# vocdoni/zk-franchise-proof-circuit

Measured on AMD Instinct MI355X. Metric: zkCensus proofs/sec (nLevels=160), higher is better.
Workload: dtype u256 (8 x u32 Montgomery, BN254 Fr/Fq)

## Files before the change

### include/zkcensus.h

```cpp
#ifndef ZKCENSUS_H
#define ZKCENSUS_H
#include <stddef.h>
#include <stdint.h>
#ifdef __cplusplus
extern "C" {
#endif

typedef struct zkc_ctx zkc_ctx;
typedef struct zkc_zkey zkc_zkey;

enum {
    ZKC_OK = 0,
    ZKC_ERR_GENERIC = 1,
    ZKC_ERR_SHORT_BUFFER = 2,
    ZKC_ERR_INVALID_WITNESS_LENGTH = 3,
    ZKC_ERR_BAD_ARG = 4,
    ZKC_ERR_FORMAT = 5,
    ZKC_ERR_HIP = 6,
    ZKC_ERR_WITNESS = 7
};
enum {
    ZKC_W_OK = 0, ZKC_W_ERR_WEIGHT = 1 , ZKC_W_ERR_SIK_ROOT = 2 ,
    ZKC_W_ERR_CENSUS_ROOT = 3 , ZKC_W_ERR_NULLIFIER = 4 , ZKC_W_ERR_LAST_SIBLING = 5 ,
    ZKC_W_ERR_INPUT_RANGE = 6 ,
// ... 5 lines not shown
void zkc_ctx_destroy(zkc_ctx* ctx);
const char* zkc_last_error(const zkc_ctx* ctx);
void* zkc_ctx_stream(zkc_ctx* ctx);

int zkc_circuit_n_inputs(int nLevels);
int zkc_circuit_n_wires(int nLevels);
int zkc_circuit_nlevels_from_wasm(const void* wasm, size_t len, char sha256_hex[65]);
void zkc_sha256(const void* data, size_t len, uint8_t out[32]);

int zkc_witness(zkc_ctx* ctx, int nLevels, const void* inputs, int B, void* wtns, int32_t* status);
int zkc_inputs_from_json(const char* json, size_t len, int nLevels, void* out, char* err, size_t errlen);
int zkc_witness_dev(zkc_ctx* ctx, int nLevels, const void* d_inputs, int B, void* d_wtns, int32_t* d_status );

int  zkc_zkey_load(zkc_ctx* ctx, const void* zkey_bytes, size_t len, zkc_zkey** out);
void zkc_zkey_free(zkc_zkey* zk);
int  zkc_zkey_info(const zkc_zkey* zk, uint32_t* nVars, uint32_t* nPublic, uint32_t* domainSize);
int  zkc_zkey_pass_info(const zkc_zkey* zk, int* pass_size, int* lanes);
int  zkc_zkey_header_info(const void* zkey_bytes, size_t len, uint32_t* nVars, uint32_t* nPublic, uint32_t* domainSize);
int  zkc_zkey_sha256(const zkc_zkey* zk, uint8_t out[32]);
int  zkc_zkey_fingerprint(const void* zkey_bytes, size_t len, uint8_t out[32]);

void zkc_random_scalars(uint8_t* out, size_t n);
int zkc_prove(zkc_zkey* zk, const void* wtns, uint32_t nWitness, const uint8_t r[32], const uint8_t s[32],
              uint8_t proof[256], uint8_t* public_out);
int zkc_prove_dev(zkc_zkey* zk, const void* d_wtns, uint32_t nWitness, const uint8_t r[32], const uint8_t s[32],
                  uint8_t proof[256], uint8_t* public_out);

int zkc_prove_batch_dev(zkc_zkey* zk, const void* d_wtns, uint32_t nWitness, int B, const uint8_t* rs, uint8_t* proofs, uint8_t* publics);

int zkc_fullprove_batch_dev(zkc_zkey* zk, const void* d_inputs, int B, void* d_wtns, int32_t* d_status, const uint8_t* rs, uint8_t* proofs, uint8_t* publics);
// ... 130 lines not shown
```

### zk-franchise-proof-circuit_amd/__init__.py

```python
import ctypes
from . import _native
from ._native import ZkcError
from .inputs import INPUT_KEYS, flatten_inputs, R_MOD

__all__ = ['Context', 'ProvingKey', 'DevicePool', 'ProvingService', 'groth16', 'ZkcError', 'INPUT_KEYS', 'flatten_inputs', 'R_MOD']


class Context:

    def __init__(self, device=0):
        self._lib = _native.load()
        h = ctypes.c_void_p()
        rc = self._lib.zkc_ctx_create(int(device), ctypes.byref(h))
        if rc != 0:
            raise ZkcError(rc, (self._lib.zkc_last_error(None) or b'').decode())
        self._h = h
        self.device = device
        self._keys = []

    def close(self):
        if getattr(self, '_h', None):
            for k in list(self._keys):
                k.close()
            self._lib.zkc_ctx_destroy(self._h)
# ... 37 lines not shown
class ProvingKey:

    def __init__(self, ctx, zkey_bytes):
        self.ctx = ctx
        self._lib = ctx._lib
        h = ctypes.c_void_p()
        ctx._check(self._lib.zkc_zkey_load(ctx._h, zkey_bytes, len(zkey_bytes), ctypes.byref(h)))
        self._h = h
        ctx._keys.append(self)
        a, b, c = ctypes.c_uint32(), ctypes.c_uint32(), ctypes.c_uint32()
        self._lib.zkc_zkey_info(h, ctypes.byref(a), ctypes.byref(b), ctypes.byref(c))
        self.n_vars, self.n_public, self.domain_size = a.value, b.value, c.value
        ps, ln = ctypes.c_int(), ctypes.c_int()
        self._lib.zkc_zkey_pass_info(h, ctypes.byref(ps), ctypes.byref(ln))
        self.pass_size, self.lanes = ps.value, ln.value

    def close(self):
        if getattr(self, '_h', None):
            if getattr(self.ctx, '_h', None):
                self._lib.zkc_zkey_free(self._h)
            self._h = None
            if self in self.ctx._keys:
                self.ctx._keys.remove(self)

    def __del__(self):
        try:
            self.close()
        except Exception:
            pass

# ... 152 lines not shown
```

### zk-franchise-proof-circuit_amd/_native.py

```python
import ctypes
import os

_HERE = os.path.dirname(os.path.abspath(__file__))
LIB_PATH = os.environ.get('ZKCENSUS_LIB') or os.path.join(_HERE, 'libzkcensus.so')
_lib = None


class ZkcError(RuntimeError):
    def __init__(self, code, msg):
        super().__init__('libzkcensus error %d: %s' % (code, msg))
        self.code = code


def load():
    global _lib
    if _lib is not None:
        return _lib
    if not os.path.exists(LIB_PATH):
        raise ImportError('libzkcensus.so is not built (run `python -c "import __graft_entry__ as g; g.build()"`); '
                          'there is no CPU fallback for the product path')
    try:
        import torch
    except ImportError:
        pass
    L = ctypes.CDLL(LIB_PATH)
    vp, i32p = ctypes.c_void_p, ctypes.POINTER(ctypes.c_int32)
    L.zkc_ctx_create.argtypes = [ctypes.c_int, ctypes.POINTER(vp)]
    L.zkc_ctx_destroy.argtypes = [vp]
    L.zkc_last_error.argtypes = [vp]; L.zkc_last_error.restype = ctypes.c_char_p
    L.zkc_ctx_stream.argtypes = [vp]; L.zkc_ctx_stream.restype = vp
    L.zkc_witness.argtypes = [vp, ctypes.c_int, vp, ctypes.c_int, vp, i32p]
    L.zkc_witness_dev.argtypes = [vp, ctypes.c_int, vp, ctypes.c_int, vp, vp]
    u8p, u32p = ctypes.c_char_p, ctypes.POINTER(ctypes.c_uint32)
    L.zkc_zkey_load.argtypes = [vp, ctypes.c_char_p, ctypes.c_size_t, ctypes.POINTER(vp)]
    L.zkc_zkey_free.argtypes = [vp]; L.zkc_zkey_free.restype = None
    L.zkc_zkey_info.argtypes = [vp, u32p, u32p, u32p]
    L.zkc_zkey_pass_info.argtypes = [vp, ctypes.POINTER(ctypes.c_int), ctypes.POINTER(ctypes.c_int)]
    L.zkc_witness_status_text.argtypes = [ctypes.c_int, ctypes.c_int32]; L.zkc_witness_status_text.restype = ctypes.c_char_p
    L.zkc_prove.argtypes = [vp, ctypes.c_char_p, ctypes.c_uint32, u8p, u8p, ctypes.c_char_p, ctypes.c_char_p]
    L.zkc_prove_dev.argtypes = [vp, vp, ctypes.c_uint32, u8p, u8p, ctypes.c_char_p, ctypes.c_char_p]
    L.zkc_prove_batch_dev.argtypes = [vp, vp, ctypes.c_uint32, ctypes.c_int, ctypes.c_char_p, ctypes.c_char_p, ctypes.c_char_p]
    L.zkc_fullprove_batch_dev.argtypes = [vp, vp, ctypes.c_int, vp, vp, ctypes.c_char_p, ctypes.c_char_p, ctypes.c_char_p]
    L.zkc_debug_stage.argtypes = [vp, vp, ctypes.c_int, ctypes.c_char_p]
    L.zkc_debug_early_retries.argtypes = []; L.zkc_debug_early_retries.restype = ctypes.c_ulonglong
    L.zkc_msm_debug.argtypes = [vp, ctypes.c_int, vp, ctypes.c_uint32, ctypes.c_char_p]
    L.zkc_debug_pairing_dev.argtypes = [vp, ctypes.c_char_p, ctypes.c_char_p, ctypes.c_char_p, ctypes.c_int, ctypes.c_char_p, ctypes.c_char_p, i32p, ctypes.POINTER(ctypes.c_int),
                                        ctypes.POINTER(ctypes.c_uint32), ctypes.c_size_t, ctypes.c_char_p]
    ulp = ctypes.POINTER(ctypes.c_ulong)
    L.groth16_prover.argtypes = [ctypes.c_char_p, ctypes.c_ulong, ctypes.c_char_p, ctypes.c_ulong, ctypes.c_char_p, ulp, ctypes.c_char_p, ulp, ctypes.c_char_p, ctypes.c_ulong]
    L.zkc_verify.argtypes = [ctypes.c_char_p, ctypes.c_char_p, ctypes.c_char_p]
    L.zkc_verify_bin.argtypes = [ctypes.c_char_p, ctypes.c_int, ctypes.c_char_p, ctypes.c_char_p]
    L.zkc_verify_batch.argtypes = [vp, ctypes.c_char_p, ctypes.c_int, ctypes.c_char_p, ctypes.c_char_p, ctypes.c_int, ctypes.c_char_p]
# ... 114 lines not shown
```

### zk-franchise-proof-circuit_amd/csrc/zkc_pass_plan.h

```cpp
#pragma once
#include "zkc_top_fold.h"
#include <cstddef>
#include <cstdint>
#include <vector>

namespace zkc {
constexpr int MSM_C_G2_LONE = 8;
constexpr int msm_nw(int c) { return (254 + c) / c; }
constexpr int msm_half(int c) { return 1 << (c - 1); }

namespace plan {

struct CallSplit { int npasses, per_pass; };
inline CallSplit call_split(int B, int max_inflight) {
    const int npasses = (B + max_inflight - 1) / max_inflight;
    return {npasses, (B + npasses - 1) / npasses};
}

constexpr int FOREIGN = -1;
inline int row_depth(const uint32_t* f, int n) {
    if (f[n - 1]) return FOREIGN;
    int D = 0; for (int g = 0; g < n - 1; g++) if (f[g]) D = g + 1;
    return D;
}
// ... 20 lines not shown
        if (!listed) seeds.push_back({q, t, slot});
    }
}

struct KeyShape {
    int c_sec, c_h, c_deep;
    uint32_t nv, np, n;
    uint32_t offA, offB1, offC, offA_deep, offB1_deep, offC_deep;
    bool lone_table, fb4;
};
struct LaneCaps { size_t w1_entries, w1_buckets; int w1_jobs; size_t w2_entries; };
struct Switches {
    uint32_t vw_big = 0, vw_small = 0, vw_g2 = 0; size_t deep_wires = 16000;
    bool matvec_inline = false, g2_acc_hold = false, g2_acc_early = false, reduce_stream = false;
    bool serial_streams = false;
};
struct PassShape {
    uint32_t vws, vwb, vw_g2;
    bool deep; int cw;
    uint32_t oA, oB1, oC;
    int c2;
    bool tree; int per;
};
template <class Lists> inline PassShape pass_shape(const KeyShape& k, int nb, const Lists* lists, const LaneCaps& cap, const Switches& s) {
    const uint32_t nv = k.nv, nc = nv - k.np - 1;
    PassShape p;
    p.vws = nb <= 4 ? 64u : s.vw_small ? s.vw_small : nb < 32 ? 256u : 2048u; p.vwb = nb <= 4 ? 256u : s.vw_big ? s.vw_big : nb < 32 ? 1024u : 4096u;
    size_t lone_entries = 0; for (int q = 0; q < nb; q++) lone_entries += (size_t)msm_nw(MSM_C_G2_LONE) * (lists ? lists[q].nB : nv);
    size_t live_wires = 0; for (int q = 0; q < nb; q++) live_wires += lists ? (size_t)lists[q].nA + lists[q].nB + lists[q].nC : 2 * (size_t)nv + nc;
    p.deep = k.c_deep != 0 && nb > 2 && live_wires >= 3 * s.deep_wires * (size_t)nb;
// ... 20 lines not shown
    bool mv_done;
    bool g2_acc_with_sort;
    bool red_split;
    bool blind_on_st;
};
inline StreamOrder stream_order(int nb, bool one_lane, int pass, int npasses, int lane0, bool tree, const Switches& s) {
    StreamOrder o;
    o.mv_prefetch = !s.matvec_inline && one_lane;
    o.mv_done = o.mv_prefetch && pass > 0;
    o.g2_acc_with_sort = s.g2_acc_hold || ((nb < 32 || !one_lane) && !s.g2_acc_early);
    o.red_split = s.reduce_stream && !s.serial_streams && nb >= 32;
    o.blind_on_st = (tree || lane0 >= 0) && npasses == 1;
    return o;
}

}}
```

### zk-franchise-proof-circuit_amd/csrc/zkc_prove.hip

```cpp
#include "zkc_prover.h"
#include "zkc_fixedbase.h"
#include "zkc_hostparse.h"
#include "zkc_host_util.h"
#include "zkc_kernels.h"
#include "zkc_f29_g2.h"
#include <cstring>
#include <ctime>
#include <cstdio>
#include <algorithm>
#include <atomic>

using namespace zkc;

void zkc::matvec_launch(zkc_zkey* zk, Fr* d_abc, Fr* d_wm, const uint32_t* d_wtns0, int nb, hipStream_t mv, const zkc_zkey::Fold::AbcRows* al) {
    const uint32_t n = zk->n, nv = zk->nVars;
    const bool units = zk->n_unit_coeffs > 0 && nv <= 3 * (size_t)n && sw::on<sw::ZKC_MATVEC_UNITS>();
    const Fr* wm = units ? (const Fr*)d_wm : (const Fr*)nullptr;
    if (al) {
        const uint32_t per = 6 * n;
        hipLaunchKernelGGL(zkc_abc_fill, dim3((per + 1023) / 1024, nb), dim3(256), 0, mv, (const uint4*)zk->fold.d_abc_tmpl, (uint4*)d_abc, per);
        if (units && al->nW) hipLaunchKernelGGL(zkc_wtns_mont_list, dim3((al->nW + 255) / 256, nb), dim3(256), 0, mv, (const Fr*)d_wtns0, (size_t)nv, d_wm, 3 * (size_t)n, al->d + al->offW, al->nW);
        if (al->nrows) hipLaunchKernelGGL(zkc_matvec_jds, dim3((al->nrows + 63 * al->nlong + 255) / 256, nb), dim3(256), 0, mv, zk->d_perm, zk->d_rowlen, zk->d_jdptr, zk->d_col, zk->d_val,
                                          (const Fr*)d_wtns0, (size_t)nv, d_abc, (int)n, al->nlong, wm, 3 * (size_t)n, (const uint32_t*)al->d, al->nrows);
        if (al->nC) hipLaunchKernelGGL(zkc_pointwise_mul, dim3((al->nC + 255) / 256, nb), dim3(256), 0, mv, d_abc, (int)n, (const uint32_t*)(al->d + al->offC), al->nC);
// ... 57 lines not shown
        lane_release(L);
        for (hipEvent_t e : {L.ev_msm, L.ev_msm2, L.ev_sorted, L.ev_ntt, L.ev_mv, L.ev_acc, L.ev_fin[0], L.ev_fin[1], L.ev_red}) if (e) (void)hipEventDestroy(e);
    }
    delete[] ctx->lanes; ctx->lanes = nullptr;
}
static int lane_init(zkc_ctx* ctx, int l) {
    zkc_lane& L = ctx_lanes(ctx)[l];
    if (L.made) return ZKC_OK;
    zkc_ctx::LaneStreams ls; int rc = zkc_lane_streams(ctx, l, sw::on<sw::ZKC_REDUCE_STREAM>(), &ls); if (rc) return rc;
    L.st = ls.st; L.st2 = ls.st2; L.fin = ls.fin; L.red = ls.red;
    for (hipEvent_t* e : {&L.ev_msm, &L.ev_msm2, &L.ev_sorted, &L.ev_ntt, &L.ev_mv, &L.ev_acc, &L.ev_fin[0], &L.ev_fin[1], &L.ev_red}) if (!*e) ZKC_HIP_CHECK(ctx, hipEventCreateWithFlags(e, hipEventDisableTiming));
    L.made = true; return ZKC_OK;
}
struct LaneSt { hipStream_t st, st2, fin, red; };
static LaneSt lane_st(const zkc_zkey* zk, const zkc_lane& L) { hipStream_t c = zk->ctx->stream; return zk->serial_streams ? LaneSt{c, c, c, c} : LaneSt{L.st, L.st2, L.fin, L.red}; }
static int lane_ensure(zkc_zkey* zk, int l, int inflight) {
    zkc_ctx* ctx = zk->ctx; int rc;
    if ((rc = lane_init(ctx, l))) return rc;
    zkc_lane& L = ctx->lanes[l];
    inflight = std::max(1, std::min(inflight, zk->max_inflight));
    if (lane_holds(L, lane_need(zk, inflight))) return ZKC_OK;
    inflight = std::min(inflight <= 4 ? 4 : zk->max_inflight, zk->max_inflight);
    LaneNeed nd = lane_need(zk, inflight);
    nd.abc = std::max(nd.abc, L.cap_abc); nd.p = std::max(nd.p, L.cap_p); nd.fin = std::max(nd.fin, L.cap_fin); nd.bs = std::max(nd.bs, L.cap_bs);
    nd.e1 = std::max(nd.e1, L.w1.max_entries); nd.b1 = std::max(nd.b1, L.w1.max_buckets); nd.j1 = std::max(nd.j1, L.w1.max_jobs);
    nd.e2 = std::max(nd.e2, L.w2.max_entries); nd.b2 = std::max(nd.b2, L.w2.max_buckets); nd.j2 = std::max(nd.j2, L.w2.max_jobs);
    for (hipStream_t q : {L.st, L.st2, L.fin, L.red}) if (q) ZKC_HIP_CHECK(ctx, hipStreamSynchronize(q));
    ZKC_HIP_CHECK(ctx, hipStreamSynchronize(ctx->stream));
    lane_release(L);
    const size_t free_before = dev_free_bytes();
// ... 129 lines not shown
    }
    {
        if (sw::on<sw::ZKC_G2_LONE_TABLE>() && (zk->nLevels >= 0 || nv < (1u << 16))) {
            if ((rc = msm_g2_window_table29(ctx, zk->d_g2, nv, MSM_C_G2_LONE, "lone-proof G2 table", &zk->d_g2_29_lone))) return bail(rc);
        }
    }
    const auto e_inf = sw::given<sw::ZKC_INFLIGHT>();
    zk->max_inflight = opt_inflight > 0 ? std::min(opt_inflight, MSM_MAX_JOBS / 4) : e_inf ? (int)*e_inf : zk->nLevels >= 0 ? 64 : 96;
    {
        const size_t per_proof_entries = (size_t)NWS * 3 * nv + (size_t)NWB * n, census_pass = 96ull * (22ull * 3 * 82754 + 15ull * 131072);
        const int fit = (int)std::max<size_t>(1, census_pass / std::max<size_t>(per_proof_entries, 1));
        zk->max_inflight = std::min(zk->max_inflight, fit);
    }
    { const auto e_l = sw::given<sw::ZKC_LANES>(); zk->nlanes = opt_lanes > 0 ? std::min(opt_lanes, (int)MAX_LANES) : e_l ? (int)*e_l : zk->nLevels >= 0 ? (int)MAX_LANES : 1; }
    zk->serial_streams = sw::on<sw::ZKC_SERIAL_STREAMS>();
    if ((rc = lanes_ensure(zk, 1, 0, 1))) return bail(rc);
    {
        FixedBase<Fq> td(zk->delta1), ta(zk->alpha1), tb(zk->beta1); FixedBase<Fq2> t2(zk->delta2);
        if ((rc = dmalloc(ctx, &zk->d_tblDelta1, td.tab.size())) || (rc = dmalloc(ctx, &zk->d_tblAlpha1, ta.tab.size())) ||
            (rc = dmalloc(ctx, &zk->d_tblBeta1, tb.tab.size())) || (rc = dmalloc(ctx, &zk->d_tblDelta2, t2.tab.size()))) return bail(rc);
        ZKC_UP(zk->d_tblDelta1, td.tab.data(), td.tab.size() * sizeof(G1Affine)); ZKC_UP(zk->d_tblAlpha1, ta.tab.data(), ta.tab.size() * sizeof(G1Affine));
        ZKC_UP(zk->d_tblBeta1, tb.tab.data(), tb.tab.size() * sizeof(G1Affine)); ZKC_UP(zk->d_tblDelta2, t2.tab.data(), t2.tab.size() * sizeof(G2Affine));
    }
    ZKC_HIP_BAIL(hipStreamSynchronize(ctx->stream));
    if (zk->nLevels >= 0 && (rc = fold_prepare(zk))) return bail(rc);
    if (zk->nLevels >= 0 && (rc = top_prepare(zk))) return bail(rc);
    if ((rc = fb4_prepare(zk))) return bail(rc);
    { const size_t f = dev_free_bytes(), grown = ctx_work_bytes(ctx) > work_at_entry ? ctx_work_bytes(ctx) - work_at_entry : 0; zk->bytes_tables = free_at_entry > f + grown ? free_at_entry - f - grown : 0; }
    *out = zk;
    return ZKC_OK;
#undef ZKC_UP
#undef ZKC_HIP_BAIL
}

int zkc::prove_reserve(zkc_zkey* zk, int inflight) {
    if (!zk) return ZKC_ERR_BAD_ARG;
    ZKC_LOCK(zk->ctx);
    ZKC_HIP_CHECK(zk->ctx, hipSetDevice(zk->ctx->device));
    return lanes_ensure(zk, inflight);
}
extern "C" int zkc_zkey_pass_info(const zkc_zkey* zk, int* pass_size, int* lanes) {
    if (!zk) return ZKC_ERR_BAD_ARG;
    if (pass_size) *pass_size = zk->max_inflight; if (lanes) *lanes = zk->nlanes;
    return ZKC_OK;
}
extern "C" int zkc_zkey_info(const zkc_zkey* zk, uint32_t* nVars, uint32_t* nPublic, uint32_t* domainSize) {
    if (!zk) return ZKC_ERR_BAD_ARG;
    if (nVars) *nVars = zk->nVars; if (nPublic) *nPublic = zk->nPub; if (domainSize) *domainSize = zk->n;
    return ZKC_OK;
}

static int h_matvec_dev(zkc_zkey* zk, zkc_lane& L, const uint32_t* d_wtns0, int nb, hipStream_t mv, const zkc_zkey::Fold::AbcRows* al = nullptr) {
    zkc_ctx* ctx = zk->ctx; const uint32_t n = zk->n, nv = zk->nVars;
    zkc_prof_scope _ps(ctx, ZKC_PROF_MATVEC, (uint64_t)nb * ((uint64_t)zk->nCoeffs * 68 + 3ull * n * 32), mv);
    matvec_launch(zk, L.d_abc, L.d_t, d_wtns0, nb, mv, al);
    ZKC_HIP_CHECK(ctx, hipGetLastError());
    return ZKC_OK;
}
// ... 134 lines not shown
            hipLaunchKernelGGL(zkc_fold_check, dim3(L.n, 2, nb), dim3(64), 0, st0, L, (const uint32_t*)wc, tmpl, fl, nb, (int)fstride);
            if (zk->fold.top.K) hipLaunchKernelGGL(zkc_top_check, dim3(2, nb), dim3(256), 0, st0, zk->fold.top.args, (const uint32_t*)wc, fl, (int)fstride, 2 * L.n);
            ZKC_HIP_CHECK(ctx, hipGetLastError());
            ZKC_HIP_CHECK(ctx, hipMemcpyAsync(CS.h_flags + (size_t)p0 * fstride, fl, (size_t)nb * fstride * 4, hipMemcpyDeviceToHost, st0));
        }
        if (CS.early_n) {
            if (d_status) ZKC_HIP_CHECK(ctx, hipMemcpyAsync(CS.h_early, d_status, 4 * (size_t)B, hipMemcpyDeviceToHost, st0));
            else memset(CS.h_early, 0, 4 * (size_t)B);
            ZKC_HIP_CHECK(ctx, hipMemcpyAsync(CS.h_early + CS.early_cap, CS.d_flags + (size_t)p0 * fstride, (size_t)nb * fstride * 4, hipMemcpyDeviceToHost, st0));
        }
        ZKC_HIP_CHECK(ctx, hipEventRecord(CS.ev_chunk[c], st0));
    }
    const bool trace_host = sw::on<sw::ZKC_TRACE_HOST>();
    auto now_ms = [] { timespec t; clock_gettime(CLOCK_MONOTONIC, &t); return t.tv_sec * 1e3 + t.tv_nsec * 1e-6; };
    const double t_begin = now_ms(); double tr[6] = {0};
    int pass = 0, done_on_st_lane = -1;
    const bool one_lane = lane0 >= 0 || zk->nlanes == 1;
    const plan::KeyShape KS{zk->c_sec, zk->c_h, zk->c_deep, nv, np, n, zk->offA, zk->offB1, zk->offC, zk->offA_deep, zk->offB1_deep, zk->offC_deep, zk->d_g2_29_lone != nullptr, zk->d_fb4 != nullptr};
    plan::Switches SW;
    SW.vw_big = (uint32_t)sw::value<sw::ZKC_VW_BIG>(0); SW.vw_small = (uint32_t)sw::value<sw::ZKC_VW_SMALL>(0); SW.vw_g2 = (uint32_t)sw::value<sw::ZKC_VW_G2>(0);
    SW.deep_wires = (size_t)sw::value<sw::ZKC_DEEP_WIRES>(16000); SW.matvec_inline = sw::on<sw::ZKC_MATVEC_INLINE>(); SW.g2_acc_hold = sw::on<sw::ZKC_G2_ACC_HOLD>();
    SW.g2_acc_early = sw::on<sw::ZKC_G2_ACC_EARLY>(); SW.reduce_stream = sw::on<sw::ZKC_REDUCE_STREAM>(); SW.serial_streams = zk->serial_streams;
    std::vector<plan::TopSeed> seeds;
    for (int p0 = 0; p0 < B; p0 += per_pass, pass++) {
        const int nb = std::min(per_pass, B - p0);
        const int li = lane0 >= 0 ? lane0 : pass % zk->nlanes; CS.lanes_used |= 1u << li;
        zkc_lane& LN = ctx->lanes[li]; const LaneSt LS = lane_st(zk, LN); const int slot = LN.npass & 1;
        tr[0] = now_ms();
        const bool early = CS.early_n > 0;
        if (!early) ZKC_HIP_CHECK(ctx, zkc_wait_event(CS.ev_chunk[pass]));
        tr[1] = now_ms();
        ZKC_HIP_CHECK(ctx, hipStreamWaitEvent(LS.st, CS.ev_chunk[pass], 0)); ZKC_HIP_CHECK(ctx, hipStreamWaitEvent(LS.st2, CS.ev_chunk[pass], 0));
        hipStream_t st = LS.st, st2 = LS.st2, fin = LS.fin;
        const uint32_t* w0 = (const uint32_t*)d_wtns + (size_t)p0 * nv * 8;
        uint8_t dcq[MSM_MAX_JOBS / 4], dsq[MSM_MAX_JOBS / 4]; bool fold = can_fold;
        if (early) for (int q = 0; q < nb; q++) { dcq[q] = CS.early_depth[2 * q]; dsq[q] = CS.early_depth[2 * q + 1]; }
        else for (int q = 0; q < nb && fold; q++) for (int t = 0; t < 2; t++) {
            const int D = plan::row_depth(CS.h_flags + (size_t)(p0 + q) * fstride + (size_t)t * L.n, L.n);
            if (D == plan::FOREIGN) { fold = false; break; }
            (t == 0 ? dcq : dsq)[q] = (uint8_t)D;
        }
        static thread_local zkc_zkey::Fold::VMap vms[MSM_MAX_JOBS / 4];
        uint16_t tcq[MSM_MAX_JOBS / 4], tsq[MSM_MAX_JOBS / 4];
        const auto& tp = zk->fold.top; const int TK = tp.K;
        plan::top_fold(dcq, dsq, CS.h_flags + (size_t)p0 * fstride + 2 * (size_t)L.n, fstride, fold ? TK : 0, tp.nslots, tp.valid.data(), early, nb, tcq, tsq, seeds);
        if (!seeds.empty() && (rc = top_seed(zk, w0, seeds))) return rc;
        if (fold) for (int q = 0; q < nb; q++) if ((rc = fold_vmap(zk, tcq[q] != top::NO_SLOT ? TK : 0, dcq[q], tsq[q] != top::NO_SLOT ? TK : 0, dsq[q], &vms[q]))) return rc;
        const bool nofold_lists = sw::on<sw::ZKC_NOFOLD_LISTS>();
        if (!fold && nofold_lists) {
            zkc_zkey::Fold::VMap nf; if ((rc = nofold_vmap(zk, &nf))) return rc;
            for (int q = 0; q < nb; q++) vms[q] = nf;
        }
        const bool listed = fold || (nofold_lists && vms[0].d != nullptr);
        if (LN.npass >= 2) { ZKC_HIP_CHECK(ctx, hipStreamWaitEvent(st, LN.ev_fin[slot], 0)); ZKC_HIP_CHECK(ctx, hipStreamWaitEvent(st2, LN.ev_fin[slot], 0)); }
        LN.npass++;
        const plan::PassShape PS = plan::pass_shape(KS, nb, listed ? vms : (const zkc_zkey::Fold::VMap*)nullptr, plan::LaneCaps{LN.w1.max_entries, LN.w1.max_buckets, LN.w1.max_jobs, LN.w2.max_entries}, SW);
        const plan::StreamOrder SO = plan::stream_order(nb, one_lane, pass, npasses, lane0, PS.tree, SW);
        const bool tree = PS.tree, mv_done = SO.mv_done;
        if (mv_done) ZKC_HIP_CHECK(ctx, hipStreamWaitEvent(st, LN.ev_mv, 0));
        zkc_zkey::Fold::AbcRows ar; const bool abc_fold = fold && !mv_done && !zk->fold.abc_cls.empty() && zk->fold.d_abc_tmpl != nullptr;
        if (abc_fold) { int Dc = 0, Ds = 0; for (int q = 0; q < nb; q++) { Dc = std::max(Dc, (int)dcq[q]); Ds = std::max(Ds, (int)dsq[q]); } if ((rc = abc_rows(zk, Dc, Ds, &ar))) return rc; }
        if ((rc = h_evals_dev(zk, LN, st, w0, nb, !mv_done, abc_fold ? &ar : nullptr))) return rc;
        ZKC_HIP_CHECK(ctx, hipEventRecord(LN.ev_ntt, st));
        tr[2] = now_ms();
        static thread_local MsmJobList j1, j2;
        j1.clear(PS.vws, PS.vwb, MSM_MAX_VW_G1); j2.clear(PS.vw_g2, 1024, MSM_MAX_VW_PER_JOB);
        for (int q = 0; q < nb; q++) j1.add(LN.d_p + 8 * (size_t)n * q, nullptr, n, zk->offH, n, 0, zk->c_h);
        auto add = [](MsmJobList& jl, const uint32_t* scalars, const plan::SectionView& v, int c) { jl.add(scalars, v.vmap, v.count, v.tbl_off, v.tbl_count, v.pt_shift, c); };
        BlindArgs ba{}; ba.rs = CS.d_rs + 64 * (size_t)p0; ba.nv = nv;
        for (int q = 0; q < nb; q++) {
            const uint32_t* w = w0 + (size_t)q * nv * 8;
            uint32_t* bs = tree ? LN.d_bs + (size_t)q * 2 * nv * 8 : nullptr;
            const plan::ProofViews v = plan::proof_views(KS, PS, w, listed ? &vms[q] : nullptr);
            add(j1, v.A.scalars, v.A, PS.cw); add(j1, v.B1.scalars, v.B1, PS.cw); add(j1, v.C.scalars, v.C, PS.cw);
            if (tree) { add(j1, bs, v.A, PS.cw); add(j1, bs + 8ull * nv, v.B1, PS.cw); }
            j2.add(w, v.B1.vmap, v.B1.count, 0, nv, 0, PS.c2);
            if (tree) { ba.w[q] = w; ba.out[q] = bs; ba.mapA[q] = v.A.vmap; ba.nA[q] = v.A.count; ba.mapB[q] = v.B1.vmap; ba.nB[q] = v.B1.count; }
        }
        if (tree && (rc = blind_scalars_launch(ctx, st, ba, nb))) return rc;
        FinalizeArgs fa{};
        fa.r1 = (const G1XYZZ*)LN.w1.results + (size_t)slot * LN.w1.max_jobs; fa.r2 = (const G2XYZZ*)LN.w2.results + (size_t)slot * LN.w2.max_jobs;
        fa.foldA = zk->fold.d_foldA; fa.foldB1 = zk->fold.d_foldB1; fa.foldC = zk->fold.d_foldC; fa.foldB2 = zk->fold.d_foldB2; fa.fold_n = can_fold ? L.n : 0;
        for (int q = 0; q < nb; q++) { fa.dc[q] = fold ? dcq[q] : (uint8_t)255; fa.ds[q] = fold ? dsq[q] : (uint8_t)255; fa.tc[q] = tcq[q]; fa.ts[q] = tsq[q]; }
        fa.topA = tp.d_A; fa.topB1 = tp.d_B1; fa.topC = tp.d_C; fa.topB2 = tp.d_B2;
        fa.tblDelta1 = zk->d_tblDelta1; fa.tblAlpha1 = zk->d_tblAlpha1; fa.tblBeta1 = zk->d_tblBeta1; fa.tblDelta2 = zk->d_tblDelta2;
        fa.alpha1 = zk->alpha1; fa.beta2 = zk->beta2; fa.rs = CS.d_rs + 64 * (size_t)p0; fa.out = CS.d_proofs + 256 * (size_t)p0; fa.scratch = LN.d_fin;
        fa.per = PS.per; fa.fb4 = zk->d_fb4; fa.fb4g2 = zk->d_fb4g2; fa.out_xyzz = CS.d_xyzz + 512 * (size_t)p0;
        const bool g2_early = !sw::on<sw::ZKC_G2_LATE>();
        auto g2_side = [&](hipEvent_t acc_after) -> int {
            if ((rc = msm_pass_g2(zk, LN.w2, j2, slot, false, st2, acc_after))) return rc;
            if (tree && (rc = finalize_tree_g2_launch(ctx, st2, fa, nb))) return rc;
            ZKC_HIP_CHECK(ctx, hipEventRecord(LN.ev_msm2, st2));
            return ZKC_OK;
        };
        if (g2_early && (rc = g2_side(SO.g2_acc_with_sort ? LN.ev_ntt : nullptr))) return rc;
        tr[3] = now_ms();
        ZKC_HIP_CHECK(ctx, hipStreamWaitEvent(st, LN.ev_red, 0));
        if ((rc = msm_pass_g1(zk, LN.w1, j1, slot, false, st, LN.ev_sorted, LN.ev_acc, (SO.red_split && LS.red) ? LS.red : nullptr, LN.ev_red))) return rc;
        tr[4] = now_ms();
        if (!g2_early) {
            ZKC_HIP_CHECK(ctx, hipStreamWaitEvent(st2, LN.ev_sorted, 0));
            if ((rc = g2_side(nullptr))) return rc;
        }
        if (want_publics)
            ZKC_HIP_CHECK(ctx, hipMemcpy2DAsync(h_pub + 32ull * np * p0, 32ull * np, w0 + 8, 32ull * nv, 32ull * np, nb, hipMemcpyDeviceToHost, st));
        ZKC_HIP_CHECK(ctx, hipEventRecord(LN.ev_msm, st));
        if (SO.mv_prefetch && p0 + per_pass < B) {
            const int p1 = p0 + per_pass, nb1 = std::min(per_pass, B - p1);
            ZKC_HIP_CHECK(ctx, hipStreamWaitEvent(fin, sw::on<sw::ZKC_MV_PREFETCH_AT_NTT>() ? LN.ev_ntt : LN.ev_sorted, 0));
            ZKC_HIP_CHECK(ctx, hipStreamWaitEvent(fin, CS.ev_chunk[pass + 1], 0));
            if ((rc = h_matvec_dev(zk, LN, (const uint32_t*)d_wtns + (size_t)p1 * nv * 8, nb1, fin))) return rc;
            ZKC_HIP_CHECK(ctx, hipEventRecord(LN.ev_mv, fin));
        }
        hipStream_t bl = SO.blind_on_st ? st : fin;
        if (bl == fin) { ZKC_HIP_CHECK(ctx, hipStreamWaitEvent(fin, LN.ev_msm, 0)); ZKC_HIP_CHECK(ctx, hipStreamWaitEvent(fin, LN.ev_red, 0)); }
        else { if (LN.npass >= 2) ZKC_HIP_CHECK(ctx, hipStreamWaitEvent(st, LN.ev_fin[slot ^ 1], 0)); if (SO.red_split) ZKC_HIP_CHECK(ctx, hipStreamWaitEvent(st, LN.ev_red, 0)); }
        if (!tree) ZKC_HIP_CHECK(ctx, hipStreamWaitEvent(bl, LN.ev_msm2, 0));
        if ((rc = finalize_launch(ctx, bl, fa, nb))) return rc;
        if (tree) ZKC_HIP_CHECK(ctx, hipStreamWaitEvent(bl, LN.ev_msm2, 0));
        if (tree) { ZKC_HIP_CHECK(ctx, hipMemcpyAsync(CS.h_xyzz + 512ull * p0, CS.d_xyzz + 512 * (size_t)p0, 512ull * nb, hipMemcpyDeviceToHost, bl)); for (int q = 0; q < nb; q++) CS.as_xyzz[p0 + q] = 1; }
        else ZKC_HIP_CHECK(ctx, hipMemcpyAsync(CS.h_out + 256ull * p0, CS.d_proofs + 256 * (size_t)p0, 256ull * nb, hipMemcpyDeviceToHost, bl));
        ZKC_HIP_CHECK(ctx, hipEventRecord(LN.ev_fin[slot], bl));
        if (bl == st) done_on_st_lane = li;
        tr[5] = now_ms();
        if (trace_host) fprintf(stderr, "[zkc host] pass %2d: start %8.2f | chunk wait %6.2f | h_evals %6.2f | g2 pass %6.2f | g1 pass %6.2f | blinding %6.2f ms\n", pass, tr[0] - t_begin,
                                tr[1] - tr[0], tr[2] - tr[1], tr[3] - tr[2], tr[4] - tr[3], tr[5] - tr[4]);
    }
    for (int l = 0; l < zk->nlanes; l++) if (CS.lanes_used >> l & 1) { const LaneSt ls = lane_st(zk, ctx->lanes[l]); ZKC_HIP_CHECK(ctx, hipEventRecord(CS.ev_done[l], done_on_st_lane == l ? ls.st : ls.fin)); }
    CS.B = B; CS.pending = true;
    return ZKC_OK;
}
static std::atomic<unsigned long long> g_early_retries{0};
extern "C" unsigned long long zkc_debug_early_retries(void) { return g_early_retries.load(); }
int zkc::prove_batch_finish(zkc_zkey* zk, int cs, uint8_t* proofs, uint8_t* publics) {
    if (!zk || !proofs || cs < 0 || cs >= CALL_SLOTS) return zkc_fail(zk ? zk->ctx : nullptr, ZKC_ERR_BAD_ARG, "prove_batch_finish: bad argument");
    zkc_zkey::CallSlot& CS = zk->call[cs];
    if (!CS.pending) return zkc_fail(zk->ctx, ZKC_ERR_BAD_ARG, "prove_batch_finish: no call in flight on this slot");
    hipError_t e = hipSuccess;
    for (int l = 0; l < zk->nlanes && e == hipSuccess; l++) if (CS.lanes_used >> l & 1) e = zkc_wait_event(CS.ev_done[l], CS.B <= 2 ? 6000u : 0u);
    CS.pending = false;
    if (e != hipSuccess) { ZKC_LOCK(zk->ctx); return zkc_fail(zk->ctx, ZKC_ERR_HIP, std::string("prove_batch_finish: ") + hipGetErrorString(e)); }
    if (CS.early_n) {
        const int n = WitnessLayout::make(zk->nLevels).n;
// ... 60 lines not shown
```

### zk-franchise-proof-circuit_amd/csrc/zkc_prover.h

```cpp
#pragma once
#include <cstring>
#include "zkc_internal.h"
#include "zkc_curve.h"
#include "zkc_abc_rows.h"
#include "zkc_top_fold.h"
#include "zkc_pass_plan.h"
#include <array>

namespace zkc {
constexpr int MSM_C_BIG = 17, MSM_C_SMALL = 12;
inline long long first_unreduced_wire(const void* w, size_t count) {
    const uint8_t* p = (const uint8_t*)w;
    for (size_t i = 0; i < count; i++) {
        uint32_t t[8]; memcpy(t, p + 32 * i, 32);
        if (t[7] >= FrParams::p[7] && !fp_std_lt_p<FrParams>(t)) return (long long)i;
    }
    return -1;
}
inline std::string unreduced_wire_msg(long long wire) { return "Witness value at wire " + std::to_string(wire) + " is not below the field order r"; }
inline int msm_c_for(size_t W) { return W < 12000 ? 12 : W < 22000 ? 13 : W < 90000 ? 15 : W < 180000 ? 16 : 17; }
constexpr int MSM_VW_MIN = 64, MSM_MAX_VW_PER_JOB = 64;
constexpr int MSM_MAX_VW_G1 = 256;
constexpr int MSM_SEG_MIN = 16;
#ifndef ZKC_MSM_SEG
// ... 111 lines not shown
    uint16_t* d_tilejob = nullptr; uint16_t* h_tilejob[2] = {nullptr, nullptr}; size_t max_tiles = 0;
    MsmJobList* h_jobs[2] = {nullptr, nullptr}; MsmWindow* h_windows[2] = {nullptr, nullptr}; hipEvent_t h_ev[2] = {nullptr, nullptr}; int h_next = 0;
    size_t max_entries = 0, max_segments = 0; int max_jobs = 0; size_t xyzz_size = 0;
};
}

struct zkc_lane {
    hipStream_t st = nullptr, st2 = nullptr, fin = nullptr;
    hipStream_t red = nullptr; hipEvent_t ev_red = nullptr;
    zkc::Fr *d_abc = nullptr, *d_t = nullptr; uint32_t* d_p = nullptr;
    void* d_fin = nullptr;
    uint32_t* d_bs = nullptr;
    zkc::MsmWork w1, w2;
    size_t cap_abc = 0, cap_p = 0, cap_fin = 0, cap_bs = 0, bytes = 0; bool made = false;
    hipEvent_t ev_msm = nullptr, ev_msm2 = nullptr, ev_sorted = nullptr, ev_ntt = nullptr, ev_mv = nullptr, ev_acc = nullptr, ev_fin[2] = {nullptr, nullptr}; int npass = 0;
};

struct zkc_zkey {
    zkc_ctx* ctx = nullptr;
    uint32_t nVars = 0, nPub = 0, n = 0, logn = 0, nCoeffs = 0;
    int nLevels = -1;
    zkc::G1Affine alpha1, beta1, delta1;
    zkc::G2Affine beta2, gamma2, delta2;
    std::vector<zkc::G1Affine> ic;
    uint32_t *d_perm = nullptr, *d_rowlen = nullptr, *d_jdptr = nullptr, *d_col = nullptr; zkc::Fr* d_val = nullptr; uint32_t nlong = 0;
    uint32_t n_unit_coeffs = 0;
    zkc::Fr *d_tw_fwd = nullptr, *d_tw_inv = nullptr, *d_coset = nullptr;
    zkc::Fr *d_coset_br = nullptr;
    uint32_t *d_tw_fwd29 = nullptr, *d_tw_inv29 = nullptr;
    zkc::G1Affine* d_g1 = nullptr; zkc::G2Affine* d_g2 = nullptr;
    uint32_t* d_g2_29 = nullptr;
    uint32_t* d_g2_29_lone = nullptr;
    uint32_t offA = 0, offB1 = 0, offC = 0, offH = 0;
    int c_deep = 0; uint32_t offA_deep = 0, offB1_deep = 0, offC_deep = 0; uint32_t* d_g2_29_deep = nullptr;
    int c_h = zkc::MSM_C_BIG;
    int c_sec = zkc::MSM_C_SMALL;
    int max_inflight = 0;
    uint8_t sha256[32] = {0};
    size_t bytes_tables = 0;
    uint8_t fingerprint[32] = {0};
    int nlanes = 1; bool serial_streams = false;
    zkc::G1Affine *d_tblDelta1 = nullptr, *d_tblAlpha1 = nullptr, *d_tblBeta1 = nullptr; zkc::G2Affine* d_tblDelta2 = nullptr;
    uint32_t *d_depths = nullptr, *h_depths = nullptr; size_t depths_cap = 0;
    zkc::G1XYZZ* d_fb4 = nullptr; zkc::G2XYZZ* d_fb4g2 = nullptr; int fb4_bases = 0;
    struct CallSlot {
        uint8_t *d_rs = nullptr, *d_proofs = nullptr; size_t cap = 0;
        uint8_t* h_out = nullptr;
        uint8_t* h_rs = nullptr;
        uint8_t *d_xyzz = nullptr, *h_xyzz = nullptr; std::vector<uint8_t> as_xyzz;
        hipEvent_t ev_done[zkc::MAX_LANES] = {};
        std::vector<hipEvent_t> ev_chunk;
        uint32_t lanes_used = 0;
        int B = 0; bool pending = false;
        uint32_t *d_flags = nullptr, *h_flags = nullptr; size_t flags_cap = 0;
        int32_t* d_status3 = nullptr; size_t status3_cap = 0;
        int early_n = 0; std::vector<uint8_t> early_depth; uint32_t* h_early = nullptr; size_t early_cap = 0;
// ... 75 lines not shown
```

### zk-franchise-proof-circuit_amd/csrc/zkc_switches.h

```cpp
#pragma once
#include <climits>
#include <cstdlib>
#include <optional>

namespace zkc { namespace sw {

enum Kind { SET, OFF_IF_ZERO, ON_IF_ONE, NUMBER, NUMBER_LONG, NUMBER_U64, TEXT };
enum When { PROCESS, LIVE };
constexpr long long ANY = LLONG_MIN;

#define ZKC_SWITCHES(X)                                                                                                                                                   \
                                                                                                                                            \
    X(ZKC_DEVICE,               TEXT,        ANY, ANY,   LIVE,    "service creation: the GPUs of the default proving service: \"2\", \"0,1,2,3\", \"all\"; unset: every visible device") \
    X(ZKC_INFLIGHT,             NUMBER,      1,   128,   LIVE,    "key load: proofs per pipeline pass (census key 64, any other 96, fewer for a large circuit); at most MSM_MAX_JOBS / 4") \
    X(ZKC_LANES,                NUMBER,      1,   4,     LIVE,    "key load: pipeline lanes the passes of a batch call rotate over (census key MAX_LANES = 4, any other 1)")      \
    X(ZKC_DEEP_TABLES,          NUMBER,      ANY, ANY,   LIVE,    "key load: 0 leaves out the second section tables that passes of deep voters take, 2 builds them for a census key of any size (default 1)") \
    X(ZKC_G2_LONE_TABLE,        OFF_IF_ZERO, ANY, ANY,   LIVE,    "key load: =0 skips the 8-bit-window G2 table of the lone-proof path")                                          \
    X(ZKC_BLIND_TREE,           OFF_IF_ZERO, ANY, ANY,   LIVE,    "key load: =0 gives a key whose passes of one or two proofs take the general blinding kernels")                 \
    X(ZKC_SERVICE_WORKERS,      NUMBER,      1,   4,     LIVE,    "service creation: workers (= lanes of a service key) per GPU (4); at most MAX_LANES")                          \
    X(ZKC_SERVICE_PASS,         NUMBER,      1,   128,   LIVE,    "service creation: proofs per pass of a service key (64); at most MSM_MAX_JOBS / 4")                            \
    X(ZKC_SERVICE_KEYS,         NUMBER,      1,   64,    LIVE,    "service creation: keys kept resident per GPU (4)")                                                             \
    X(ZKC_SERVICE_MAX_BATCH,    NUMBER,      1,   4096,  LIVE,    "service creation: requests one worker takes per call (256)")                                                   \
    X(ZKC_SERVICE_MIN_BATCH,    NUMBER,      1,   ANY,   LIVE,    "service creation: requests a collecting worker waits for before it goes (16)")                                 \
    X(ZKC_SERVICE_SPILL,        NUMBER,      1,   ANY,   LIVE,    "service creation: queue length at which a cold GPU is brought up (32)")                                        \
    X(ZKC_SERVICE_BUSY_WAIT_US, NUMBER,      0,   ANY,   LIVE,    "service creation: microseconds a collecting worker waits for more requests (300)")                             \
    X(ZKC_SERVICE_RESERVE,      OFF_IF_ZERO, ANY, ANY,   PROCESS, "=0: a service key load does not reserve a full pass of work space on every lane; the lanes grow on demand")    \
    X(ZKC_DEVICE_BLOCKING_SYNC, ON_IF_ONE,   ANY, ANY,   LIVE,    "context creation: =1 asks HIP for blocking waits on the device (hipDeviceScheduleBlockingSync)")               \
    X(ZKC_SPIN_WAIT,            SET,         ANY, ANY,   PROCESS, "set (any value, 0 included): host waits use hipEventSynchronize instead of polling with short sleeps")         \
    X(ZKC_VERIFY_BATCH_GPU,     NUMBER,      ANY, ANY,   LIVE,    "per verify call: 0 keeps the Miller loops of zkc_verify_batch on the host, positive forces the GPU, negative or unset: GPU from 128 proofs") \
    X(ZKC_NO_SHA_NI,            SET,         ANY, ANY,   PROCESS, "set (any value, 0 included): portable SHA-256 instead of the CPU's SHA extensions")                            \
// ... 82 lines not shown
```

Baseline: 3390.

## Collapse per-lane pass streams onto one stream when rotating over lanes

When a batch call rotates passes over several lanes, each pass now puts G1, G2 and blinding work on the lane's single G1 stream by default. A new switch still allows two or three streams. Same-stream event waits and records are skipped, and done/fin events track which stream they were recorded on. The aim is to cut cross-stream event overhead and stream contention, since the lanes already give concurrency. The cost is less overlap of G2 MSM and blinding within a lane.

```diff
diff --git a/include/zkcensus.h b/include/zkcensus.h
--- a/include/zkcensus.h
+++ b/include/zkcensus.h
@@ -43,6 +43,7 @@
 
 int  zkc_zkey_load(zkc_ctx* ctx, const void* zkey_bytes, size_t len, zkc_zkey** out);
 void zkc_zkey_free(zkc_zkey* zk);
+int  zkc_zkey_call_streams(const zkc_zkey* zk, int* streams);
 int  zkc_zkey_info(const zkc_zkey* zk, uint32_t* nVars, uint32_t* nPublic, uint32_t* domainSize);
 int  zkc_zkey_pass_info(const zkc_zkey* zk, int* pass_size, int* lanes);
 int  zkc_zkey_header_info(const void* zkey_bytes, size_t len, uint32_t* nVars, uint32_t* nPublic, uint32_t* domainSize);
diff --git a/zk-franchise-proof-circuit_amd/__init__.py b/zk-franchise-proof-circuit_amd/__init__.py
--- a/zk-franchise-proof-circuit_amd/__init__.py
+++ b/zk-franchise-proof-circuit_amd/__init__.py
@@ -75,6 +75,11 @@
         ps, ln = ctypes.c_int(), ctypes.c_int()
         self._lib.zkc_zkey_pass_info(h, ctypes.byref(ps), ctypes.byref(ln))
         self.pass_size, self.lanes = ps.value, ln.value
+
+    def call_streams(self):
+        n = ctypes.c_int()
+        self.ctx._check(self._lib.zkc_zkey_call_streams(self._h, ctypes.byref(n)))
+        return n.value
 
     def close(self):
         if getattr(self, '_h', None):
diff --git a/zk-franchise-proof-circuit_amd/_native.py b/zk-franchise-proof-circuit_amd/_native.py
--- a/zk-franchise-proof-circuit_amd/_native.py
+++ b/zk-franchise-proof-circuit_amd/_native.py
@@ -36,6 +36,7 @@
     L.zkc_zkey_free.argtypes = [vp]; L.zkc_zkey_free.restype = None
     L.zkc_zkey_info.argtypes = [vp, u32p, u32p, u32p]
     L.zkc_zkey_pass_info.argtypes = [vp, ctypes.POINTER(ctypes.c_int), ctypes.POINTER(ctypes.c_int)]
+    L.zkc_zkey_call_streams.argtypes = [vp, ctypes.POINTER(ctypes.c_int)]
     L.zkc_witness_status_text.argtypes = [ctypes.c_int, ctypes.c_int32]; L.zkc_witness_status_text.restype = ctypes.c_char_p
     L.zkc_prove.argtypes = [vp, ctypes.c_char_p, ctypes.c_uint32, u8p, u8p, ctypes.c_char_p, ctypes.c_char_p]
     L.zkc_prove_dev.argtypes = [vp, vp, ctypes.c_uint32, u8p, u8p, ctypes.c_char_p, ctypes.c_char_p]
diff --git a/zk-franchise-proof-circuit_amd/csrc/zkc_pass_plan.h b/zk-franchise-proof-circuit_amd/csrc/zkc_pass_plan.h
--- a/zk-franchise-proof-circuit_amd/csrc/zkc_pass_plan.h
+++ b/zk-franchise-proof-circuit_amd/csrc/zkc_pass_plan.h
@@ -58,6 +58,7 @@
     uint32_t vw_big = 0, vw_small = 0, vw_g2 = 0; size_t deep_wires = 16000;
     bool matvec_inline = false, g2_acc_hold = false, g2_acc_early = false, reduce_stream = false;
     bool serial_streams = false;
+    int lane_streams = 0;
 };
 struct PassShape {
     uint32_t vws, vwb, vw_g2;
@@ -108,4 +109,25 @@
     return o;
 }
 
+enum LaneStream { ON_ST = 0, ON_ST2 = 1, ON_FIN = 2, ON_RED = 3 };
+struct LaneRoles {
+    int g1;
+    int g2;
+    int blind;
+    int red;
+    int streams;
+};
+inline LaneRoles lane_roles(int nb, bool one_lane, int pass, int npasses, int lane0, bool tree, int lanes, const Switches& s) {
+    const StreamOrder o = stream_order(nb, one_lane, pass, npasses, lane0, tree, s);
+    const bool rotates = !one_lane && lanes > 1;
+    const int want = !rotates ? 3 : (s.lane_streams >= 1 && s.lane_streams <= 3) ? s.lane_streams : 1;
+    LaneRoles r;
+    r.g1 = ON_ST;
+    r.g2 = want >= 2 ? ON_ST2 : ON_ST;
+    r.blind = (o.blind_on_st || want <= 2) ? ON_ST : ON_FIN;
+    r.red = o.red_split ? ON_RED : ON_ST;
+    r.streams = 1 + (r.g2 != ON_ST) + (r.blind != ON_ST) + (r.red != ON_ST);
+    return r;
+}
+
 }}
diff --git a/zk-franchise-proof-circuit_amd/csrc/zkc_prove.hip b/zk-franchise-proof-circuit_amd/csrc/zkc_prove.hip
--- a/zk-franchise-proof-circuit_amd/csrc/zkc_prove.hip
+++ b/zk-franchise-proof-circuit_amd/csrc/zkc_prove.hip
@@ -95,6 +95,9 @@
 }
 struct LaneSt { hipStream_t st, st2, fin, red; };
 static LaneSt lane_st(const zkc_zkey* zk, const zkc_lane& L) { hipStream_t c = zk->ctx->stream; return zk->serial_streams ? LaneSt{c, c, c, c} : LaneSt{L.st, L.st2, L.fin, L.red}; }
+struct PassSt { hipStream_t st, st2, bl, red; };
+static PassSt pass_st(const LaneSt& s, const plan::LaneRoles& r) { const hipStream_t by[4] = {s.st, s.st2, s.fin, s.red}; return PassSt{by[r.g1], by[r.g2], by[r.blind], by[r.red] ? by[r.red] : by[r.g1]}; }
+static hipError_t wait_unless_same(hipStream_t s, hipEvent_t e, hipStream_t on) { return (!on || on == s) ? hipSuccess : hipStreamWaitEvent(s, e, 0); }
 static int lane_ensure(zkc_zkey* zk, int l, int inflight) {
     zkc_ctx* ctx = zk->ctx; int rc;
     if ((rc = lane_init(ctx, l))) return rc;
@@ -254,6 +257,7 @@
     }
     { const auto e_l = sw::given<sw::ZKC_LANES>(); zk->nlanes = opt_lanes > 0 ? std::min(opt_lanes, (int)MAX_LANES) : e_l ? (int)*e_l : zk->nLevels >= 0 ? (int)MAX_LANES : 1; }
     zk->serial_streams = sw::on<sw::ZKC_SERIAL_STREAMS>();
+    zk->lane_streams = (int)sw::value<sw::ZKC_LANE_STREAMS>(0);
     if ((rc = lanes_ensure(zk, 1, 0, 1))) return bail(rc);
     {
         FixedBase<Fq> td(zk->delta1), ta(zk->alpha1), tb(zk->beta1); FixedBase<Fq2> t2(zk->delta2);
@@ -282,6 +286,12 @@
 extern "C" int zkc_zkey_pass_info(const zkc_zkey* zk, int* pass_size, int* lanes) {
     if (!zk) return ZKC_ERR_BAD_ARG;
     if (pass_size) *pass_size = zk->max_inflight; if (lanes) *lanes = zk->nlanes;
+    return ZKC_OK;
+}
+extern "C" int zkc_zkey_call_streams(const zkc_zkey* zk, int* streams) {
+    if (!zk || !streams) return ZKC_ERR_BAD_ARG;
+    ZKC_LOCK(zk->ctx);
+    *streams = zk->last_call_streams;
     return ZKC_OK;
 }
 extern "C" int zkc_zkey_info(const zkc_zkey* zk, uint32_t* nVars, uint32_t* nPublic, uint32_t* domainSize) {
@@ -446,13 +456,17 @@
     const bool trace_host = sw::on<sw::ZKC_TRACE_HOST>();
     auto now_ms = [] { timespec t; clock_gettime(CLOCK_MONOTONIC, &t); return t.tv_sec * 1e3 + t.tv_nsec * 1e-6; };
     const double t_begin = now_ms(); double tr[6] = {0};
-    int pass = 0, done_on_st_lane = -1;
+    int pass = 0;
+    hipStream_t done_on[MAX_LANES] = {};
+    hipStream_t touched[1 + 4 * MAX_LANES] = {st0}; int ntouched = 1;
+    auto touch = [&](hipStream_t s) { for (int i = 0; i < ntouched; i++) if (touched[i] == s) return; touched[ntouched++] = s; };
     const bool one_lane = lane0 >= 0 || zk->nlanes == 1;
+    const int lanes = lane0 >= 0 ? 1 : std::min(zk->nlanes, npasses);
     const plan::KeyShape KS{zk->c_sec, zk->c_h, zk->c_deep, nv, np, n, zk->offA, zk->offB1, zk->offC, zk->offA_deep, zk->offB1_deep, zk->offC_deep, zk->d_g2_29_lone != nullptr, zk->d_fb4 != nullptr};
     plan::Switches SW;
     SW.vw_big = (uint32_t)sw::value<sw::ZKC_VW_BIG>(0); SW.vw_small = (uint32_t)sw::value<sw::ZKC_VW_SMALL>(0); SW.vw_g2 = (uint32_t)sw::value<sw::ZKC_VW_G2>(0);
     SW.deep_wires = (size_t)sw::value<sw::ZKC_DEEP_WIRES>(16000); SW.matvec_inline = sw::on<sw::ZKC_MATVEC_INLINE>(); SW.g2_acc_hold = sw::on<sw::ZKC_G2_ACC_HOLD>();
-    SW.g2_acc_early = sw::on<sw::ZKC_G2_ACC_EARLY>(); SW.reduce_stream = sw::on<sw::ZKC_REDUCE_STREAM>(); SW.serial_streams = zk->serial_streams;
+    SW.g2_acc_early = sw::on<sw::ZKC_G2_ACC_EARLY>(); SW.reduce_stream = sw::on<sw::ZKC_REDUCE_STREAM>(); SW.serial_streams = zk->serial_streams; SW.lane_streams = zk->lane_streams;
     std::vector<plan::TopSeed> seeds;
     for (int p0 = 0; p0 < B; p0 += per_pass, pass++) {
         const int nb = std::min(per_pass, B - p0);
@@ -462,8 +476,6 @@
         const bool early = CS.early_n > 0;
         if (!early) ZKC_HIP_CHECK(ctx, zkc_wait_event(CS.ev_chunk[pass]));
         tr[1] = now_ms();
-        ZKC_HIP_CHECK(ctx, hipStreamWaitEvent(LS.st, CS.ev_chunk[pass], 0)); ZKC_HIP_CHECK(ctx, hipStreamWaitEvent(LS.st2, CS.ev_chunk[pass], 0));
-        hipStream_t st = LS.st, st2 = LS.st2, fin = LS.fin;
         const uint32_t* w0 = (const uint32_t*)d_wtns + (size_t)p0 * nv * 8;
         uint8_t dcq[MSM_MAX_JOBS / 4], dsq[MSM_MAX_JOBS / 4]; bool fold = can_fold;
         if (early) for (int q = 0; q < nb; q++) { dcq[q] = CS.early_depth[2 * q]; dsq[q] = CS.early_depth[2 * q + 1]; }
@@ -484,16 +496,20 @@
             for (int q = 0; q < nb; q++) vms[q] = nf;
         }
         const bool listed = fold || (nofold_lists && vms[0].d != nullptr);
-        if (LN.npass >= 2) { ZKC_HIP_CHECK(ctx, hipStreamWaitEvent(st, LN.ev_fin[slot], 0)); ZKC_HIP_CHECK(ctx, hipStreamWaitEvent(st2, LN.ev_fin[slot], 0)); }
-        LN.npass++;
         const plan::PassShape PS = plan::pass_shape(KS, nb, listed ? vms : (const zkc_zkey::Fold::VMap*)nullptr, plan::LaneCaps{LN.w1.max_entries, LN.w1.max_buckets, LN.w1.max_jobs, LN.w2.max_entries}, SW);
         const plan::StreamOrder SO = plan::stream_order(nb, one_lane, pass, npasses, lane0, PS.tree, SW);
+        const PassSt PT = pass_st(LS, plan::lane_roles(nb, one_lane, pass, npasses, lane0, PS.tree, lanes, SW));
+        const hipStream_t st = PT.st, st2 = PT.st2, bl = PT.bl, fin = LS.fin;
+        touch(st); touch(st2); touch(bl); touch(PT.red);
+        ZKC_HIP_CHECK(ctx, hipStreamWaitEvent(st, CS.ev_chunk[pass], 0)); if (st2 != st) ZKC_HIP_CHECK(ctx, hipStreamWaitEvent(st2, CS.ev_chunk[pass], 0));
+        if (LN.npass >= 2) { ZKC_HIP_CHECK(ctx, wait_unless_same(st, LN.ev_fin[slot], LN.fin_on[slot])); if (st2 != st) ZKC_HIP_CHECK(ctx, wait_unless_same(st2, LN.ev_fin[slot], LN.fin_on[slot])); }
+        LN.npass++;
         const bool tree = PS.tree, mv_done = SO.mv_done;
         if (mv_done) ZKC_HIP_CHECK(ctx, hipStreamWaitEvent(st, LN.ev_mv, 0));
         zkc_zkey::Fold::AbcRows ar; const bool abc_fold = fold && !mv_done && !zk->fold.abc_cls.empty() && zk->fold.d_abc_tmpl != nullptr;
         if (abc_fold) { int Dc = 0, Ds = 0; for (int q = 0; q < nb; q++) { Dc = std::max(Dc, (int)dcq[q]); Ds = std::max(Ds, (int)dsq[q]); } if ((rc = abc_rows(zk, Dc, Ds, &ar))) return rc; }
         if ((rc = h_evals_dev(zk, LN, st, w0, nb, !mv_done, abc_fold ? &ar : nullptr))) return rc;
-        ZKC_HIP_CHECK(ctx, hipEventRecord(LN.ev_ntt, st));
+        if (st2 != st || SO.mv_prefetch) ZKC_HIP_CHECK(ctx, hipEventRecord(LN.ev_ntt, st));
         tr[2] = now_ms();
         static thread_local MsmJobList j1, j2;
         j1.clear(PS.vws, PS.vwb, MSM_MAX_VW_G1); j2.clear(PS.vw_g2, 1024, MSM_MAX_VW_PER_JOB);
@@ -520,23 +536,27 @@
         fa.per = PS.per; fa.fb4 = zk->d_fb4; fa.fb4g2 = zk->d_fb4g2; fa.out_xyzz = CS.d_xyzz + 512 * (size_t)p0;
         const bool g2_early = !sw::on<sw::ZKC_G2_LATE>();
         auto g2_side = [&](hipEvent_t acc_after) -> int {
+            if (LN.g2_done) ZKC_HIP_CHECK(ctx, wait_unless_same(st2, LN.g2_done, LN.g2_on));
             if ((rc = msm_pass_g2(zk, LN.w2, j2, slot, false, st2, acc_after))) return rc;
             if (tree && (rc = finalize_tree_g2_launch(ctx, st2, fa, nb))) return rc;
-            ZKC_HIP_CHECK(ctx, hipEventRecord(LN.ev_msm2, st2));
+            if (st2 != bl) ZKC_HIP_CHECK(ctx, hipEventRecord(LN.ev_msm2, st2));
+            LN.g2_on = st2; LN.g2_done = st2 != bl ? LN.ev_msm2 : LN.ev_fin[slot];
             return ZKC_OK;
         };
-        if (g2_early && (rc = g2_side(SO.g2_acc_with_sort ? LN.ev_ntt : nullptr))) return rc;
+        if (g2_early && (rc = g2_side(SO.g2_acc_with_sort && st2 != st ? LN.ev_ntt : nullptr))) return rc;
         tr[3] = now_ms();
-        ZKC_HIP_CHECK(ctx, hipStreamWaitEvent(st, LN.ev_red, 0));
-        if ((rc = msm_pass_g1(zk, LN.w1, j1, slot, false, st, LN.ev_sorted, LN.ev_acc, (SO.red_split && LS.red) ? LS.red : nullptr, LN.ev_red))) return rc;
+        ZKC_HIP_CHECK(ctx, wait_unless_same(st, LN.ev_red, LN.red_on));
+        const bool want_sorted = SO.mv_prefetch || (!g2_early && st2 != st);
+        if ((rc = msm_pass_g1(zk, LN.w1, j1, slot, false, st, want_sorted ? LN.ev_sorted : nullptr, PT.red != st ? LN.ev_acc : nullptr, PT.red != st ? PT.red : nullptr, LN.ev_red))) return rc;
+        LN.red_on = PT.red;
         tr[4] = now_ms();
         if (!g2_early) {
-            ZKC_HIP_CHECK(ctx, hipStreamWaitEvent(st2, LN.ev_sorted, 0));
+            if (st2 != st) ZKC_HIP_CHECK(ctx, hipStreamWaitEvent(st2, LN.ev_sorted, 0));
             if ((rc = g2_side(nullptr))) return rc;
         }
         if (want_publics)
             ZKC_HIP_CHECK(ctx, hipMemcpy2DAsync(h_pub + 32ull * np * p0, 32ull * np, w0 + 8, 32ull * nv, 32ull * np, nb, hipMemcpyDeviceToHost, st));
-        ZKC_HIP_CHECK(ctx, hipEventRecord(LN.ev_msm, st));
+        if (bl != st) ZKC_HIP_CHECK(ctx, hipEventRecord(LN.ev_msm, st));
         if (SO.mv_prefetch && p0 + per_pass < B) {
             const int p1 = p0 + per_pass, nb1 = std::min(per_pass, B - p1);
             ZKC_HIP_CHECK(ctx, hipStreamWaitEvent(fin, sw::on<sw::ZKC_MV_PREFETCH_AT_NTT>() ? LN.ev_ntt : LN.ev_sorted, 0));
@@ -544,21 +564,22 @@
             if ((rc = h_matvec_dev(zk, LN, (const uint32_t*)d_wtns + (size_t)p1 * nv * 8, nb1, fin))) return rc;
             ZKC_HIP_CHECK(ctx, hipEventRecord(LN.ev_mv, fin));
         }
-        hipStream_t bl = SO.blind_on_st ? st : fin;
-        if (bl == fin) { ZKC_HIP_CHECK(ctx, hipStreamWaitEvent(fin, LN.ev_msm, 0)); ZKC_HIP_CHECK(ctx, hipStreamWaitEvent(fin, LN.ev_red, 0)); }
-        else { if (LN.npass >= 2) ZKC_HIP_CHECK(ctx, hipStreamWaitEvent(st, LN.ev_fin[slot ^ 1], 0)); if (SO.red_split) ZKC_HIP_CHECK(ctx, hipStreamWaitEvent(st, LN.ev_red, 0)); }
-        if (!tree) ZKC_HIP_CHECK(ctx, hipStreamWaitEvent(bl, LN.ev_msm2, 0));
+        if (bl != st) ZKC_HIP_CHECK(ctx, hipStreamWaitEvent(bl, LN.ev_msm, 0));
+        ZKC_HIP_CHECK(ctx, wait_unless_same(bl, LN.ev_red, LN.red_on));
+        if (LN.npass >= 2) ZKC_HIP_CHECK(ctx, wait_unless_same(bl, LN.ev_fin[slot ^ 1], LN.fin_on[slot ^ 1]));
+        if (!tree && st2 != bl) ZKC_HIP_CHECK(ctx, hipStreamWaitEvent(bl, LN.ev_msm2, 0));
         if ((rc = finalize_launch(ctx, bl, fa, nb))) return rc;
-        if (tree) ZKC_HIP_CHECK(ctx, hipStreamWaitEvent(bl, LN.ev_msm2, 0));
+        if (tree && st2 != bl) ZKC_HIP_CHECK(ctx, hipStreamWaitEvent(bl, LN.ev_msm2, 0));
         if (tree) { ZKC_HIP_CHECK(ctx, hipMemcpyAsync(CS.h_xyzz + 512ull * p0, CS.d_xyzz + 512 * (size_t)p0, 512ull * nb, hipMemcpyDeviceToHost, bl)); for (int q = 0; q < nb; q++) CS.as_xyzz[p0 + q] = 1; }
         else ZKC_HIP_CHECK(ctx, hipMemcpyAsync(CS.h_out + 256ull * p0, CS.d_proofs + 256 * (size_t)p0, 256ull * nb, hipMemcpyDeviceToHost, bl));
-        ZKC_HIP_CHECK(ctx, hipEventRecord(LN.ev_fin[slot], bl));
-        if (bl == st) done_on_st_lane = li;
+        ZKC_HIP_CHECK(ctx, hipEventRecord(LN.ev_fin[slot], bl)); LN.fin_on[slot] = bl;
+        done_on[li] = bl;
         tr[5] = now_ms();
         if (trace_host) fprintf(stderr, "[zkc host] pass %2d: start %8.2f | chunk wait %6.2f | h_evals %6.2f | g2 pass %6.2f | g1 pass %6.2f | blinding %6.2f ms\n", pass, tr[0] - t_begin,
                                 tr[1] - tr[0], tr[2] - tr[1], tr[3] - tr[2], tr[4] - tr[3], tr[5] - tr[4]);
     }
-    for (int l = 0; l < zk->nlanes; l++) if (CS.lanes_used >> l & 1) { const LaneSt ls = lane_st(zk, ctx->lanes[l]); ZKC_HIP_CHECK(ctx, hipEventRecord(CS.ev_done[l], done_on_st_lane == l ? ls.st : ls.fin)); }
+    for (int l = 0; l < zk->nlanes; l++) if (CS.lanes_used >> l & 1) ZKC_HIP_CHECK(ctx, hipEventRecord(CS.ev_done[l], done_on[l]));
+    zk->last_call_streams = ntouched;
     CS.B = B; CS.pending = true;
     return ZKC_OK;
 }
diff --git a/zk-franchise-proof-circuit_amd/csrc/zkc_prover.h b/zk-franchise-proof-circuit_amd/csrc/zkc_prover.h
--- a/zk-franchise-proof-circuit_amd/csrc/zkc_prover.h
+++ b/zk-franchise-proof-circuit_amd/csrc/zkc_prover.h
@@ -149,6 +149,8 @@
     zkc::MsmWork w1, w2;
     size_t cap_abc = 0, cap_p = 0, cap_fin = 0, cap_bs = 0, bytes = 0; bool made = false;
     hipEvent_t ev_msm = nullptr, ev_msm2 = nullptr, ev_sorted = nullptr, ev_ntt = nullptr, ev_mv = nullptr, ev_acc = nullptr, ev_fin[2] = {nullptr, nullptr}; int npass = 0;
+    hipStream_t g2_on = nullptr; hipEvent_t g2_done = nullptr;
+    hipStream_t fin_on[2] = {nullptr, nullptr}, red_on = nullptr;
 };
 
 struct zkc_zkey {
@@ -175,6 +177,8 @@
     size_t bytes_tables = 0;
     uint8_t fingerprint[32] = {0};
     int nlanes = 1; bool serial_streams = false;
+    int lane_streams = 0;
+    int last_call_streams = 0;
     zkc::G1Affine *d_tblDelta1 = nullptr, *d_tblAlpha1 = nullptr, *d_tblBeta1 = nullptr; zkc::G2Affine* d_tblDelta2 = nullptr;
     uint32_t *d_depths = nullptr, *h_depths = nullptr; size_t depths_cap = 0;
     zkc::G1XYZZ* d_fb4 = nullptr; zkc::G2XYZZ* d_fb4g2 = nullptr; int fb4_bases = 0;
diff --git a/zk-franchise-proof-circuit_amd/csrc/zkc_switches.h b/zk-franchise-proof-circuit_amd/csrc/zkc_switches.h
--- a/zk-franchise-proof-circuit_amd/csrc/zkc_switches.h
+++ b/zk-franchise-proof-circuit_amd/csrc/zkc_switches.h
@@ -14,6 +14,7 @@
     X(ZKC_DEVICE,               TEXT,        ANY, ANY,   LIVE,    "service creation: the GPUs of the default proving service: \"2\", \"0,1,2,3\", \"all\"; unset: every visible device") \
     X(ZKC_INFLIGHT,             NUMBER,      1,   128,   LIVE,    "key load: proofs per pipeline pass (census key 64, any other 96, fewer for a large circuit); at most MSM_MAX_JOBS / 4") \
     X(ZKC_LANES,                NUMBER,      1,   4,     LIVE,    "key load: pipeline lanes the passes of a batch call rotate over (census key MAX_LANES = 4, any other 1)")      \
+    X(ZKC_LANE_STREAMS,         NUMBER,      1,   3,     LIVE,    "key load: streams of a lane that a pass of a call rotating over several lanes uses: 1 all on the G1 stream (default), 2 the G2 MSM on its own, 3 the blinding too") \
     X(ZKC_DEEP_TABLES,          NUMBER,      ANY, ANY,   LIVE,    "key load: 0 leaves out the second section tables that passes of deep voters take, 2 builds them for a census key of any size (default 1)") \
     X(ZKC_G2_LONE_TABLE,        OFF_IF_ZERO, ANY, ANY,   LIVE,    "key load: =0 skips the 8-bit-window G2 table of the lone-proof path")                                          \
     X(ZKC_BLIND_TREE,           OFF_IF_ZERO, ANY, ANY,   LIVE,    "key load: =0 gives a key whose passes of one or two proofs take the general blinding kernels")                 \
```

Result: faster. 3459 (median of 6 runs) (+2.0%).
